# xxcclong/GNN-Computing

Hardware: AMD Instinct MI355X
Metric: aggregated edges/sec, GCN SpMM feat=128 (higher is better)
Workload: dtype f32; 1 GPU; arxiv-shaped CSR 169343x1166243 (seed 123), GCN sum, feat=128, unit weights, locality reorder applied on load (.reorder_thres_0.2), mode=balanced; num_v=169343, num_e=1166243, feat=128

## Files before the change

gnn_computing_amd/csrc/agg_gcn.hip:

```cpp
#include "combine.cuh"

namespace gnnagg {

template <int VEC, int GROUP, bool IS_MAX, bool LIST>
__device__ __forceinline__ void gcn_items_body(const GcnArgs &a)
{
    constexpr int ITEMS = block_of<GROUP>() / GROUP;
    const int b = logical_block(blockIdx.x, a.nblocks, a.ntiles, a.remap, a.xr);
    if (b < 0) return;
    const int tile = b % a.ntiles;
    const int item = (b / a.ntiles) * ITEMS + (int)threadIdx.x / GROUP;
    const int lane = threadIdx.x & (GROUP - 1);
    const int col = (tile * GROUP + lane) * VEC;
    if (item >= a.n_total) return;
    const bool col_ok = col < a.feat;
    const int F = a.feat;

    if (LIST && item >= a.n_items) {
        const float z[VEC] = {};
        if (col_ok) store_pack<VEC>(a.y + (size_t)a.empty_rows[item - a.n_items] * F + col, z);
        return;
    }
    const int beg = a.ptr[item], end = a.ptr[item + 1];
    float acc[VEC];
// ... 119 lines not shown
    const int F = a.feat;
    const int slot = ~d.z;
    if (grp == 0 && col_ok) store_pack_wt<VEC>(a.partial, a.partial_bytes, (size_t)slot * F + col, acc);
    asm volatile("s_waitcnt vmcnt(0) lgkmcnt(0)" ::: "memory");
    __shared__ int s_hub;
    __syncthreads();
    if (threadIdx.x == 0) {
        const int m = a.slot_hub[slot];
        const int nseg = a.mrow_ptr[m + 1] - a.mrow_ptr[m];
        int *cnt = a.hub_count + (size_t)m * a.hub_count_stride + tile;
        const int old = __hip_atomic_fetch_add(cnt, 1, __ATOMIC_RELAXED, __HIP_MEMORY_SCOPE_AGENT);
        if (old == nseg - 1) __hip_atomic_store(cnt, 0, __ATOMIC_RELAXED, __HIP_MEMORY_SCOPE_AGENT);
        s_hub = old == nseg - 1 ? m : -1;
    }
    __syncthreads();
    const int m = s_hub;
    if (m < 0) return false;
    const int s0 = a.mrow_ptr[m], s1 = a.mrow_ptr[m + 1];
    const int row = a.mrow_id[m];
    row_out = row;
#pragma unroll
    for (int k = 0; k < VEC; ++k) acc[k] = IS_MAX ? -INFINITY : 0.0f;
    for (int sb = s0; sb < s1; sb += kSegChunks) {
        const int nst = s1 - sb < kSegChunks ? s1 - sb : kSegChunks;
        for (int p = grp; p < nst; p += GPB)
            if (col_ok) {
                const Pack<VEC> v = load_pack_sc1<VEC>(a.partial, a.partial_bytes, (size_t)(sb + p) * F + col);
                store_pack<VEC>(&stage[(p * GROUP + lane) * VEC], v.v);
            }
        __syncthreads();
        if (grp == 0 && col_ok) {
#pragma unroll
            for (int p = 0; p < kSegChunks; ++p)
                if (p < nst) {
                    const Pack<VEC> v = load_pack<VEC>(&stage[(p * GROUP + lane) * VEC]);
#pragma unroll
                    for (int k = 0; k < VEC; ++k) {
                        if (IS_MAX) acc[k] = v.v[k] > acc[k] ? v.v[k] : acc[k];
                        else acc[k] += v.v[k];
                    }
                }
        }
        __syncthreads();
    }
    if (grp == 0 && col_ok) {
        finish_gcn_row<VEC, IS_MAX>(acc, a.mean ? a.row_ptr[row + 1] - a.row_ptr[row] : 1, row, a.y + (size_t)row * F + col, a.mean,
                                    a.accumulate, a.relu, a.row_aux, TYPED ? a.yvec : VEC);
        if constexpr (TYPED) store_y_typed<VEC>(a.y, a.y_bf16, a.yvec, 0, 0, (size_t)row * F + col, acc);
        else store_pack<VEC>(a.y + (size_t)row * F + col, acc);
    }
    return true;
}

#ifdef GNNAGG_PLAN_WAVES
#define PLAN_WAVES_ATTR __attribute__((amdgpu_waves_per_eu(GNNAGG_PLAN_WAVES, GNNAGG_PLAN_WAVES)))
#else
#define PLAN_WAVES_ATTR
#endif
template <int VEC, int GROUP, bool IS_MAX, bool PROBE = false, int UNROLL = kUnroll, typename TX = float, bool TYPED = false>
__global__ __launch_bounds__(block_of<GROUP>()) PLAN_WAVES_ATTR void k_gcn_plan(const PlanArgs a)
{
    static_assert(TYPED || std::is_same<TX, float>::value, "16-bit X needs the typed store");
    constexpr int GPB = block_of<GROUP>() / GROUP;
    const int F = a.feat;
    const int lane = threadIdx.x & (GROUP - 1);
    const int grp = (int)threadIdx.x / GROUP;
    const int nb1 = a.n1 * a.ntiles;
    if (PROBE && (int)blockIdx.x < nb1) {
        const int tile = (int)blockIdx.x % a.ntiles;
        const int4 d = a.t1[(int)blockIdx.x / a.ntiles];
        const int col = (tile * GROUP + lane) * VEC;
        const int nch = (d.y - d.x + a.chunk - 1) / a.chunk;
        unsigned sig = 0;
        for (int c = grp; c < nch; c += GPB) {
            const int cb = d.x + c * a.chunk;
            const int ce = cb + a.chunk < d.y ? cb + a.chunk : d.y;
            sig ^= probe_edges<VEC, GROUP, UNROLL>(cb, ce, lane, col < F, a.idx, a.val, a.x + col, F);
        }
        if (sig == 0x9e3779b9u) a.probe_sink[0] = sig;
        return;
    }
    if ((int)blockIdx.x < nb1) {
        __shared__ float stage[kSegChunks * GROUP * VEC];
        const int tile = (int)blockIdx.x % a.ntiles;
        const int4 d = a.t1[(int)blockIdx.x / a.ntiles];
        const int col = (tile * GROUP + lane) * VEC;
        const bool col_ok = col < F;
        const int nch = (d.y - d.x + a.chunk - 1) / a.chunk;
        for (int c = grp; c < nch; c += GPB) {
            float acc[VEC];
#pragma unroll
            for (int k = 0; k < VEC; ++k) acc[k] = IS_MAX ? -INFINITY : 0.0f;
            const int cb = d.x + c * a.chunk;
            const int ce = cb + a.chunk < d.y ? cb + a.chunk : d.y;
            chain_edges<VEC, GROUP, IS_MAX, UNROLL, TX>(acc, cb, ce, lane, col_ok, a.idx, a.val, reinterpret_cast<const TX *>(a.x) + col, F);
            store_pack<VEC>(&stage[(c * GROUP + lane) * VEC], acc);
        }
        __syncthreads();
        const bool hub_here = d.z < 0 && a.hub_count != nullptr;
        if (!hub_here && (grp != 0 || !col_ok)) return;
        float acc[VEC];
#pragma unroll
        for (int k = 0; k < VEC; ++k) acc[k] = IS_MAX ? -INFINITY : 0.0f;
        if (grp == 0 && col_ok) {
#pragma unroll
            for (int c = 0; c < kSegChunks; ++c)
                if (c < nch) {
                    const Pack<VEC> p = load_pack<VEC>(&stage[(c * GROUP + lane) * VEC]);
#pragma unroll
                    for (int k = 0; k < VEC; ++k) {
                        if (IS_MAX) acc[k] = p.v[k] > acc[k] ? p.v[k] : acc[k];
                        else acc[k] += p.v[k];
                    }
                }
        }
        if (hub_here) {
            int row;
            hub_arrive_and_fold<VEC, GROUP, IS_MAX, TYPED>(a, d, tile, col, col_ok, grp, lane, acc, stage, row);
        } else if (d.z >= 0) {
            finish_gcn_row<VEC, IS_MAX>(acc, d.y - d.x, d.z, a.y + (size_t)d.z * F + col, a.mean, a.accumulate, a.relu, a.row_aux,
                                        TYPED ? a.yvec : VEC);
            if constexpr (TYPED) store_y_typed<VEC>(a.y, a.y_bf16, a.yvec, 0, 0, (size_t)d.z * F + col, acc);
            else store_pack<VEC>(a.y + (size_t)d.z * F + col, acc);
        } else {
            store_pack<VEC>(a.partial + (size_t)(~d.z) * F + col, acc);
        }
        return;
    }
    const int b = a.tile_major ? logical_block_tile_major((int)blockIdx.x - nb1, a.item_blocks, a.ntiles, a.xr)
                               : logical_block((int)blockIdx.x - nb1, a.nblocks0, a.ntiles, a.remap, a.xr);
    if (b < 0) return;
    const int tile = b % a.ntiles;
    const int item = (b / a.ntiles) * GPB + grp;
    if (item >= a.n0) return;
    const int col = (tile * GROUP + lane) * VEC;
    const bool col_ok = col < F;
    const int4 d = a.t0[item];
    const TX *__restrict__ xcol = reinterpret_cast<const TX *>(a.x) + (size_t)tile * a.x_tile_stride + lane * VEC;
    if constexpr (PROBE) {
        const unsigned sig = probe_edges<VEC, GROUP, UNROLL>(d.x, d.y, lane, col_ok, a.idx, a.val, xcol, a.xpitch);
        if (sig == 0x9e3779b9u) a.probe_sink[0] = sig;
        return;
    }
    if (a.accumulate && !a.relu && d.x == d.y) return;
    float acc[VEC];
#pragma unroll
    for (int k = 0; k < VEC; ++k) acc[k] = IS_MAX ? -INFINITY : 0.0f;
    chain_edges<VEC, GROUP, IS_MAX, UNROLL, TX>(acc, d.x, d.y, lane, col_ok, a.idx, a.val, xcol, a.xpitch);
    if (!col_ok) return;
    if (d.z < 0) {
        const size_t poff = (size_t)(~d.z) * a.ppitch + lane * VEC;
        if (a.ptile_bytes) store_pack_wt<VEC>(a.partial + (size_t)tile * a.p_tile_stride, a.ptile_bytes, poff, acc);
        else store_pack<VEC>(a.partial + (size_t)tile * a.p_tile_stride + poff, acc);
        return;
    }
    if (d.x == d.y) {
#pragma unroll
        for (int k = 0; k < VEC; ++k) acc[k] = 0.0f;
        finish_gcn_row<VEC, false>(acc, 1, d.z, a.y + (size_t)d.z * F + col, 0, a.accumulate, a.relu, nullptr, TYPED ? a.yvec : VEC);
    } else {
        finish_gcn_row<VEC, IS_MAX>(acc, d.y - d.x, d.z, a.y + (size_t)d.z * F + col, a.mean, a.accumulate, a.relu, a.row_aux,
                                    TYPED ? a.yvec : VEC);
    }
    if constexpr (TYPED) store_y_typed<VEC>(a.y, a.y_bf16, a.yvec, a.wt, a.ybytes, (size_t)d.z * F + col, acc);
    else if (a.yvec < VEC || F - col < VEC) store_pack_any<VEC>(a.y + (size_t)d.z * F + col, acc, F - col, a.yvec);
    else if (a.wt) store_pack_wt<VEC>(a.y, a.ybytes, (size_t)d.z * F + col, acc);
    else store_pack<VEC>(a.y + (size_t)d.z * F + col, acc);
}

#ifndef NN_ROWS
#define NN_ROWS 16
#endif
static constexpr int kNnRows = NN_ROWS;

struct NnArgs {
    const float *weight;
    float *out;
    int n_out;
};

template <int KB, int ROWS>
__device__ __forceinline__ void tile_times_weight(const float *tile, int pitch, const int *tile_rows, const float *W, int K,
                                                  int Kw, int N, float *out)
{
    const int wave = (int)threadIdx.x >> 6, lane = (int)threadIdx.x & 63;
    const int ncb = (N + 15) >> 4;
    const int Kf = K & ~3;
    const int kq = lane >> 4;
    const __amdgpu_buffer_rsrc_t wrsrc = __builtin_amdgcn_make_buffer_rsrc(const_cast<float *>(W), 0, Kw * N * 4, 0x00020000);
    bool synced = false;
    constexpr int RH = ROWS / 16;
// ... 524 lines not shown
            if (is_max) hipLaunchKernelGGL((k_gcn_plan<VEC, GROUP, true, false, 4, TX, true>), dim3(grid), dim3(blk), 0, stream, a);
            else        hipLaunchKernelGGL((k_gcn_plan<VEC, GROUP, false, false, 4, TX, true>), dim3(grid), dim3(blk), 0, stream, a);
            return;
        }
    }
    if (is_max) hipLaunchKernelGGL((k_gcn_plan<VEC, GROUP, true, false, kUnroll, TX, true>), dim3(grid), dim3(blk), 0, stream, a);
    else        hipLaunchKernelGGL((k_gcn_plan<VEC, GROUP, false, false, kUnroll, TX, true>), dim3(grid), dim3(blk), 0, stream, a);
}

int launch_gcn_plan(const GcnPlanLaunch &L, void *stream_v)
{
    hipStream_t stream = (hipStream_t)stream_v;
    if (L.feat <= 0) return fail(GNNAGG_ERR_ARG, "feature length must be >= 1");
    if (L.tile.on && (L.n1 > 0 || L.accumulate)) return fail(GNNAGG_ERR_STATE, "internal: tiled launch with segments");
    const bool typed = L.x_dtype != GNNAGG_DTYPE_F32 || L.y_dtype != GNNAGG_DTYPE_F32;
    if (typed && (L.tile.on || L.probe || L.nn_weight || L.t0_partials))
        return fail(GNNAGG_ERR_STATE, "internal: typed launch on a path without 16-bit forms");
    const int xsize = L.x_dtype == GNNAGG_DTYPE_BF16 ? 2 : 4, ysize = L.y_dtype == GNNAGG_DTYPE_BF16 ? 2 : 4;
    const Geometry g = L.tile.on ? tile_geometry(L.tile, L.feat)
                       : typed   ? typed_geometry(L.feat, L.x, xsize)
                                 : pick_geometry(L.feat, L.x, L.y, L.partial, L.feat);
    const bool is_max = L.reduce == GNNAGG_REDUCE_MAX;
    PlanArgs a;
    a.t0 = reinterpret_cast<const int4 *>(L.t0); a.t1 = reinterpret_cast<const int4 *>(L.t1);
    a.idx = L.idx; a.val = L.val; a.x = static_cast<const float *>(L.x); a.y = static_cast<float *>(L.y); a.partial = L.partial;
    a.n0 = L.n0; a.n1 = L.n1; a.feat = L.feat; a.ntiles = g.ntiles; a.chunk = L.chunk;
    a.mean = L.reduce == GNNAGG_REDUCE_MEAN; a.remap = L.xcd_remap; a.accumulate = L.accumulate; a.relu = L.relu;
    a.row_aux = L.row_aux;
    a.slot_hub = L.slot_hub; a.mrow_ptr = L.hubs.mrow_ptr; a.mrow_id = L.hubs.mrow_id; a.row_ptr = L.row_ptr;
    a.hub_count = L.hub_count; a.hub_count_stride = L.hub_count_stride; a.partial_bytes = 0;
    a.xpitch = L.feat; a.ppitch = L.feat; a.x_tile_stride = a.p_tile_stride = g.group * g.vec;
    a.yvec = typed ? align_class(L.feat, L.y, ysize, g.vec) : g.vec;
    a.y_bf16 = L.y_dtype == GNNAGG_DTYPE_BF16 ? 1 : 0;
    a.tile_major = 0; a.item_blocks = 0; a.ptile_bytes = 0; a.probe_sink = nullptr;
    if (L.tile.on) {
        a.xpitch = L.tile.xpitch; a.x_tile_stride = L.tile.x_tile_stride; a.ppitch = L.tile.ppitch;
        a.p_tile_stride = L.tile.p_tile_stride; a.yvec = L.tile.yvec; a.tile_major = 1;
        const size_t tb = (size_t)L.hubs.n_slots * L.tile.ppitch * sizeof(float);
        a.ptile_bytes = tb < 0x7fffffffULL ? (unsigned)tb : 0u;
    }
    {
        const size_t pbytes = (size_t)L.hubs.n_slots * L.feat * sizeof(float);
        if (L.hubs.n_mrows == 0 || pbytes >= 0x7fffffffULL || g.ntiles > L.hub_count_stride) a.hub_count = nullptr;
        else a.partial_bytes = (unsigned)pbytes;
    }
    const bool hubs_in_kernel = a.hub_count != nullptr;
    {
        const size_t ybytes = (size_t)L.num_rows * L.feat * ysize;
        a.wt = (!L.accumulate && ybytes < 0x7fffffffULL && g.vec * ysize <= 16) ? 1 : 0;
        a.ybytes = (unsigned)ybytes;
    }
    const bool want_nn = L.nn_weight != nullptr;
    const bool fuse_nn = want_nn && !L.tile.on && !L.probe && g.ntiles == 1 && g.group >= 16 && !L.accumulate && !L.relu && !L.t0_partials;
    const bool u4 = L.unroll == 4 && g.vec == 4 && (g.group == 32 || g.group == 64) && !L.tile.on && !fuse_nn;
    const int blk = block_for(g.group);
    const int gpb = fuse_nn ? std::max(kNnRows, blk / g.group) : blk / g.group;
    const int item_blocks = ceil_div(a.n0, gpb);
    a.nblocks0 = item_blocks * g.ntiles;
    a.item_blocks = item_blocks;
    if (a.remap && a.nblocks0 < 64 && !a.tile_major) a.remap = 0;
    int grid0 = a.nblocks0;
    if (a.tile_major) {
        if (!L.t0_cost_prefix) return fail(GNNAGG_ERR_STATE, "internal: tiled launch without item costs");
        grid0 = 8 * fill_xcd_ranges_tile_major(L.t0_cost_prefix, a.n0, gpb, item_blocks, g.ntiles, a.xr);
    } else if (a.remap == 2) {
        if (!L.t0_cost_prefix) a.remap = 1;
        else grid0 = 8 * fill_xcd_ranges(L.t0_cost_prefix, a.n0, gpb, item_blocks, a.xr) * g.ntiles;
    }
    const int grid = a.n1 * g.ntiles + grid0;
    if (typed) {
        if (grid > 0) {
            const bool u4t = L.unroll == 4 && g.vec * xsize == 16 && g.group >= 32;
#define CALL_TYPED(TXT) launch_plan_typed<VEC, GROUP, TXT>(a, is_max, u4t, grid, blk, stream)
            if (L.x_dtype == GNNAGG_DTYPE_BF16) {
                DISPATCH_GEOM_16BIT(g, CALL_TYPED(__bf16))
            } else {
                DISPATCH_GEOM(g, CALL_TYPED(float))
            }
#undef CALL_TYPED
            HIP_TRY(hipGetLastError());
        }
        if (hubs_in_kernel) return GNNAGG_OK;
        GcnLaunch C;
        C.wl = L.hubs; C.row_ptr = L.row_ptr; C.y = static_cast<float *>(L.y); C.partial = L.partial; C.feat = L.feat; C.reduce = L.reduce;
        C.accumulate = L.accumulate; C.relu = L.relu; C.row_aux = L.row_aux;
        if (L.y_dtype == GNNAGG_DTYPE_F32) return launch_combine_gcn(C, pick_geometry(L.feat, L.partial, L.y, nullptr, L.feat), is_max, stream);
        const int cv = align_class(L.feat, L.y, ysize, 4);
        return launch_combine_gcn(C, Geometry{cv, 64, ceil_div(L.feat, 64 * cv)}, is_max, stream, nullptr, nullptr, 0, nullptr, true);
    }
    if (L.probe) {
        if (is_max) return fail(GNNAGG_ERR_ARG, "probe: sum/mean only");
        a.probe_sink = device_probe_sink();
        if (!a.probe_sink) return fail(GNNAGG_ERR_HIP, "probe: no sink");
        if (grid > 0) {
#define CALL_PROBE hipLaunchKernelGGL((k_gcn_plan<VEC, GROUP, false, true>), dim3(grid), dim3(blk), 0, stream, a);
            if (u4 && g.group == 32) hipLaunchKernelGGL((k_gcn_plan<4, 32, false, true, 4>), dim3(grid), dim3(blk), 0, stream, a);
            else if (u4) hipLaunchKernelGGL((k_gcn_plan<4, 64, false, true, 4>), dim3(grid), dim3(blk), 0, stream, a);
            else DISPATCH_GEOM(g, CALL_PROBE)
#undef CALL_PROBE
            HIP_TRY(hipGetLastError());
        }
        return GNNAGG_OK;
    }
    if (fuse_nn) {
        NnArgs w;
        w.weight = L.nn_weight; w.out = L.nn_out; w.n_out = L.nn_cols;
        if (grid > 0) {
#define CALL_PLAN_NN                                                                                                 \
            if (is_max) hipLaunchKernelGGL((k_gcn_plan_nn<VEC, GROUP, true>), dim3(grid), dim3(blk), 0, stream, a, w);     \
            else        hipLaunchKernelGGL((k_gcn_plan_nn<VEC, GROUP, false>), dim3(grid), dim3(blk), 0, stream, a, w);
            DISPATCH_GEOM(g, CALL_PLAN_NN)
#undef CALL_PLAN_NN
            HIP_TRY(hipGetLastError());
        }
        GcnLaunch C;
        C.wl = L.hubs; C.row_ptr = L.row_ptr; C.y = static_cast<float *>(L.y); C.partial = L.partial; C.feat = L.feat; C.reduce = L.reduce;
        if (hubs_in_kernel) return GNNAGG_OK;
        return launch_combine_gcn(C, g, is_max, stream, L.nn_weight, L.nn_out, L.nn_cols);
    }
    if (grid > 0) {
#define CALL_PLAN                                                                                            \
        if (is_max) hipLaunchKernelGGL((k_gcn_plan<VEC, GROUP, true>), dim3(grid), dim3(blk), 0, stream, a);        \
        else        hipLaunchKernelGGL((k_gcn_plan<VEC, GROUP, false>), dim3(grid), dim3(blk), 0, stream, a);
        if (u4 && g.group == 32) {
            if (is_max) hipLaunchKernelGGL((k_gcn_plan<4, 32, true, false, 4>), dim3(grid), dim3(blk), 0, stream, a);
            else        hipLaunchKernelGGL((k_gcn_plan<4, 32, false, false, 4>), dim3(grid), dim3(blk), 0, stream, a);
        } else if (u4) {
            if (is_max) hipLaunchKernelGGL((k_gcn_plan<4, 64, true, false, 4>), dim3(grid), dim3(blk), 0, stream, a);
            else        hipLaunchKernelGGL((k_gcn_plan<4, 64, false, false, 4>), dim3(grid), dim3(blk), 0, stream, a);
        } else DISPATCH_GEOM(g, CALL_PLAN)
#undef CALL_PLAN
        HIP_TRY(hipGetLastError());
    }
    GcnLaunch C;
    C.wl = L.hubs; C.row_ptr = L.row_ptr; C.y = static_cast<float *>(L.y); C.partial = L.partial; C.feat = L.feat; C.reduce = L.reduce;
    C.accumulate = L.accumulate; C.relu = L.relu; C.row_aux = L.row_aux;
    const int rc = hubs_in_kernel ? GNNAGG_OK : launch_combine_gcn(C, g, is_max, stream, nullptr, nullptr, 0, &L.tile);
    if (rc || !want_nn) return rc;
    return launch_dense_nn(static_cast<const float *>(L.y), L.nn_weight, L.nn_out, L.num_rows, L.nn_cols, L.feat, stream);
}

int launch_gcn_rows_long(const GcnRowsLongLaunch &L, void *stream_v)
{
    hipStream_t stream = (hipStream_t)stream_v;
    if (L.n1 <= 0) return GNNAGG_OK;
    auto aligned = [](const void *p, size_t al) { return ((uintptr_t)p % al) == 0; };
    int vec = 1;
    if (L.feat % 4 == 0 && aligned(L.x, 16)) vec = 4;
    else if (L.feat % 2 == 0 && aligned(L.x, 8)) vec = 2;
    RowsLongArgs a;
    a.r1 = reinterpret_cast<const int4 *>(L.r1); a.idx = L.idx; a.val = L.val; a.x = L.x; a.y = L.y;
    a.n1 = L.n1; a.feat = L.feat; a.ntiles = ceil_div(L.feat, 32); a.mean = L.reduce == GNNAGG_REDUCE_MEAN; a.relu = L.relu;
    a.att = L.att; a.heads = L.heads; a.dhead = L.heads > 0 ? L.feat / L.heads : L.feat; a.slope = L.slope;
    const bool is_max = L.reduce == GNNAGG_REDUCE_MAX;
    const bool is_gat = L.att != nullptr;
    if (is_gat && (a.dhead % 32) != 0) return fail(GNNAGG_ERR_ARG, "long-row GAT kernel needs head width % 32 == 0");
    const bool wide = !L.medium && !is_gat && L.feat > 32 && (L.tile_w == 64 || (L.tile_w == 0 && (long)a.n1 * a.ntiles > 2L * device_cu_count()));
    if (wide) a.ntiles = ceil_div(L.feat, 64);
    const int grid = a.n1 * a.ntiles;
#define LAUNCH_LONG(V, B)                                                                                            \
    {                                                                                                                \
        const size_t lds = (size_t)long_round_edges<V, B>() * (2 * 32 + 2) * sizeof(float);                          \
        if (is_gat)      LAUNCH_LONG_K((k_gcn_rows_long<V, false, true, B>), B)                                      \
        else if (is_max) LAUNCH_LONG_K((k_gcn_rows_long<V, true, false, B>), B)                                      \
        else             LAUNCH_LONG_K((k_gcn_rows_long<V, false, false, B>), B)                                     \
    }
#define LAUNCH_WIDE(V)                                                                                               \
    {                                                                                                                \
        const size_t lds = (size_t)long_round_edges<V, kLongBlock, 64>() * (2 * 64 + 2) * sizeof(float);             \
        if (is_max) LAUNCH_LONG_K((k_gcn_rows_long<V, true, false, kLongBlock, 64>), kLongBlock)                     \
        else        LAUNCH_LONG_K((k_gcn_rows_long<V, false, false, kLongBlock, 64>), kLongBlock)                    \
    }
#define LAUNCH_LONG_K(K, B)                                                                                          \
    {                                                                                                                \
        static OncePerDevice big_lds_ok;  \
        if (lds > 64 * 1024 && big_lds_ok.first()) {                                                                 \
            HIP_TRY(hipFuncSetAttribute(reinterpret_cast<const void *>(&K), hipFuncAttributeMaxDynamicSharedMemorySize, (int)lds)); \
            big_lds_ok.done();                                                                                       \
        }                                                                                                            \
        hipLaunchKernelGGL(K, dim3(grid), dim3(B), lds, stream, a);                                                  \
    }
    if (!L.medium && !is_gat && !wide && vec == 4) {
// ... 67 lines not shown
```

gnn_computing_amd/csrc/api.hip:

```cpp
#include <hip/hip_runtime.h>

#include <algorithm>
#include <cstdio>
#include <cstdlib>
#include <cstring>
#include <ctime>
#include <mutex>
#include <queue>
#include <set>
#include <vector>

#include "api_internal.h"

namespace gnnagg {

static thread_local std::string g_last_error;
static bool g_abort_on_error = true;

int fail(int code, const std::string &msg)
{
    g_last_error = msg;
    return code;
}

// ... 138 lines not shown
                                    h_val.empty() ? nullptr : s.h_val_s.data(), tgt.data(), keep_eid ? eid.data() : nullptr);
    ptr_s.resize((size_t)G + 1);
    tgt.resize((size_t)G);
    const int kept = ptr_s[G];
    if (keep_eid) {
        eid.resize((size_t)kept);
        int rc2 = s.eperm.upload(eid);
        if (rc2) return rc2;
        if (c->keep_h_eperm) s.h_eperm = eid;
    }
    s.h_idx_s.resize((size_t)kept);
    if (!s.h_val_s.empty()) s.h_val_s.resize((size_t)kept);
    s.h_ptr_s.swap(ptr_s);
    s.h_target.swap(tgt);
    return finalize_schedule(c, s);
}

static int build_plan_into(Ctx *c, BalancedPlan &p, int chunk, bool describe_in_sched1, double *padding_ratio)
{
    int rc = fetch_host_ptr(c);
    if (rc) return rc;
    p.reset();
    p.chunk = chunk;
    const int V = c->V;
    const long seg_edges = (long)chunk * kSegChunksHost;
    std::vector<int> t0, t1, mrow_id, mrow_ptr(1, 0), big;
    struct Seg { int beg, end, dest, row; };
    std::vector<Seg> segs;
    p.t0_cost_prefix.assign(1, 0);
    int nslots = 0;
    for (int r = 0; r < V; ++r) {
        const int beg = c->h_ptr[r], end = c->h_ptr[r + 1], deg = end - beg;
        if (deg <= chunk) {
            t0.insert(t0.end(), {beg, end, r, r});
            p.t0_cost_prefix.push_back(p.t0_cost_prefix.back() + deg + kItemCost);
        } else if (deg <= seg_edges) {
            segs.push_back({beg, end, r, r});
        } else {
            const int nseg = (int)((deg + seg_edges - 1) / seg_edges);
            for (int j = 0; j < nseg; ++j) {
                const long sb = beg + (long)j * seg_edges;
                segs.push_back({(int)sb, (int)std::min<long>(sb + seg_edges, end), ~(nslots + j), r});
            }
            if (nseg > kBigRowPartials) big.push_back((int)mrow_id.size());
            nslots += nseg;
            mrow_id.push_back(r);
            mrow_ptr.push_back(nslots);
        }
    }
    std::stable_sort(segs.begin(), segs.end(), [](const Seg &a, const Seg &b) { return a.end - a.beg > b.end - b.beg; });
    for (const Seg &sg : segs) t1.insert(t1.end(), {sg.beg, sg.end, sg.dest, sg.row});
    p.n0 = (int)(t0.size() / 4);
    p.n1 = (int)(t1.size() / 4);
    p.n_mrows = (int)mrow_id.size();
    p.n_slots = nslots;
    p.n_big = (int)big.size();
    if ((rc = p.t0.upload(t0))) return rc;
    p.h_t0 = t0;
    if ((rc = p.t1.upload(t1))) return rc;
    if ((rc = p.mrow_id.upload(mrow_id))) return rc;
    if ((rc = p.mrow_ptr.upload(mrow_ptr))) return rc;
    if ((rc = p.big_rows.upload(big))) return rc;
    {
        std::vector<int> slot_hub((size_t)nslots);
        for (size_t m = 0; m + 1 < mrow_ptr.size(); ++m)
            for (int sl = mrow_ptr[m]; sl < mrow_ptr[m + 1]; ++sl) slot_hub[sl] = (int)m;
        if ((rc = p.slot_hub.upload(slot_hub))) return rc;
    }
    if (padding_ratio) {
        long padded = 0, chunks = p.n0;
        for (const Seg &sg : segs) {
            const long nch = ((long)sg.end - sg.beg + chunk - 1) / chunk;
            padded += 8 * ((nch + 7) / 8);
            chunks += nch;
        }
        *padding_ratio = chunks > 0 ? (double)(padded + p.n0) / (double)chunks : 1.0;
    }
    if (describe_in_sched1) {
        Schedule &s = c->sched[1];
        s.reset();
        s.kind = GNNAGG_SCHED_NEIGHBOR_GROUPING;
        const int G = neighbor_grouping(c->h_ptr.data(), chunk, V, nullptr, nullptr);
        s.h_ptr_s.resize((size_t)G + 1);
        s.h_target.resize((size_t)G);
        neighbor_grouping(c->h_ptr.data(), chunk, V, s.h_ptr_s.data(), s.h_target.data());
        s.num_target = G;
    }
    p.valid = true;
    return GNNAGG_OK;
}

static int build_balanced_plan(Ctx *c, int chunk) { return build_plan_into(c, c->plan, chunk, true, nullptr); }
static int pick_chunk(const Ctx *c);
static int build_balanced_plan_keep(Ctx *c) { return build_plan_into(c, c->plan, pick_chunk(c), false, nullptr); }

#ifndef GNNAGG_SORT_ROW_BYTES
#define GNNAGG_SORT_ROW_BYTES 256
#endif
static bool wants_sorted_rows(const Ctx *c, long row_bytes) { return c->sort_window > 1 && row_bytes <= GNNAGG_SORT_ROW_BYTES; }

static int ensure_sorted_rows(Ctx *c, BalancedPlan &p)
{
    if (p.t0_sorted.p || p.n0 == 0) return GNNAGG_OK;
    const int n0 = p.n0;
    const std::vector<int> &t0 = p.h_t0;
    std::vector<int> order((size_t)n0);
// ... 625 lines not shown
        S.span_g = rb.span_g.p + s0; S.n_spans = s1 - s0; S.span_cost_prefix = rb.cost[(size_t)p].data();
        if ((rc = launch_gat_span(G, c->stream))) return rc;
    }
    if ((rc = launch_untile_y_gat(c->yt.p, c->den_t.p, y, rb.n1 > 0 ? rb.hub_mask.p : nullptr, c->V, feat, tr.spec.tile_w, ht, dhead, c->stream))) return rc;
    if (fork) HIP_TRY(hipStreamWaitEvent(c->stream, c->ev_join, 0));
    else if (rb.n1 > 0 && (rc = hub_rows(c->stream))) return rc;
    *used = true;
    return GNNAGG_OK;
}

int gcn_run(Ctx *c, const float *x, float *y, int feat, int mode, int reduce, int flags, const NnRequest *nn, int probe, int x_dtype,
            int y_dtype)
{
    const bool typed = x_dtype != GNNAGG_DTYPE_F32 || y_dtype != GNNAGG_DTYPE_F32;
    if (typed && (nn || probe)) return fail(GNNAGG_ERR_ARG, "16-bit features: run_with_nn and the gather probe are fp32 only");
    if ((flags & GNNAGG_FLAG_ACCUMULATE) && (mode != GNNAGG_MODE_BALANCED || (reduce != GNNAGG_REDUCE_SUM && !c->row_aux) || !c->use_plan))
        return fail(GNNAGG_ERR_ARG, "GNNAGG_FLAG_ACCUMULATE needs GNNAGG_MODE_BALANCED and GNNAGG_REDUCE_SUM (mean / max: gnnagg_set_row_aux first)");
    const bool aux_run = c->row_aux != nullptr && reduce != GNNAGG_REDUCE_SUM;
    if (aux_run && (mode != GNNAGG_MODE_BALANCED || !c->use_plan || nn || probe))
        return fail(GNNAGG_ERR_ARG, "gnnagg_set_row_aux applies to plain GNNAGG_MODE_BALANCED runs only");
    if (c->kind != Ctx::GCN) return fail(GNNAGG_ERR_ARG, "handle is not a GCN aggregator");
    if ((flags & GNNAGG_FLAG_RELU) && nn) return fail(GNNAGG_ERR_ARG, "GNNAGG_FLAG_RELU is not available in run_with_nn");
    if (flags & ~(GNNAGG_FLAG_ACCUMULATE | GNNAGG_FLAG_RELU)) return fail(GNNAGG_ERR_ARG, "unknown flag bits");
    if (!x || !y) return fail(GNNAGG_ERR_ARG, "null feature pointer");
    if (reduce < GNNAGG_REDUCE_SUM || reduce > GNNAGG_REDUCE_MAX) return fail(GNNAGG_ERR_ARG, "bad reduce");
    if (mode < GNNAGG_MODE_ROWS || mode > GNNAGG_MODE_BALANCED) return fail(GNNAGG_ERR_ARG, "bad mode");
    if (mode == GNNAGG_MODE_ROWS && c->fast_rows) mode = GNNAGG_MODE_BALANCED;
    if (mode == GNNAGG_MODE_SCHEDULED && c->fast_scheduled && c->sched[0].valid && sched_keeps_every_edge(c)) mode = GNNAGG_MODE_BALANCED;
    if (mode == GNNAGG_MODE_ROWS && c->opt_rows_blocked && c->tiled && c->use_plan && reduce != GNNAGG_REDUCE_MAX && !probe) {
        bool used = false;
        const int rcb = run_rows_blocked(c, x, y, feat, reduce, flags, nn, &used);
        if (rcb || used) return rcb;
    }
    Schedule *s = nullptr;
    int rc = get_sched(c, mode, &s);
    if (rc) return rc;
    const bool acc_on_partitioned = ((flags & GNNAGG_FLAG_ACCUMULATE) || aux_run || typed) && c->partitions > 0;
    const bool on_plan = (mode == GNNAGG_MODE_BALANCED && c->use_plan && (c->partitions == 0 || acc_on_partitioned)) ||
                         (mode == GNNAGG_MODE_SCHEDULED && c->plan_sched.valid);
    if (typed && !on_plan)
        return fail(GNNAGG_ERR_ARG, std::string("gnnagg_gcn_run_typed (x ") + (x_dtype == GNNAGG_DTYPE_BF16 ? "bf16" : "fp32") + ", y " +
                                        (y_dtype == GNNAGG_DTYPE_BF16 ? "bf16" : "fp32") +
                                        "): this order runs on the item kernels, which are fp32 only -- use GNNAGG_MODE_BALANCED, or a "
                                        "neighbor-grouping schedule / \"fast_scheduled\" = 1 for GNNAGG_MODE_SCHEDULED");
    if (acc_on_partitioned && !c->plan.valid && (rc = build_balanced_plan_keep(c))) return rc;
    if (on_plan) {
        BalancedPlan &p = mode == GNNAGG_MODE_BALANCED ? c->plan : c->plan_sched;
        GcnPlanLaunch P;
        P.t0 = p.t0.p; P.t1 = p.t1.p; P.n0 = p.n0; P.n1 = p.n1; P.chunk = p.chunk;
        P.t0_cost_prefix = p.t0_cost_prefix.data();
        if (wants_sorted_rows(c, (long)feat * (x_dtype == GNNAGG_DTYPE_BF16 ? 2 : 4))) {
            if ((rc = ensure_sorted_rows(c, p))) return rc;
            if (p.t0_sorted.p) { P.t0 = p.t0_sorted.p; P.t0_cost_prefix = p.t0s_cost_prefix.data(); }
        }
        P.hubs.mrow_id = p.mrow_id.p; P.hubs.mrow_ptr = p.mrow_ptr.p; P.hubs.n_mrows = p.n_mrows;
        P.hubs.n_slots = p.n_slots; P.hubs.big_rows = p.big_rows.p; P.hubs.n_big = p.n_big;
        P.row_ptr = c->d_ptr; P.idx = c->d_idx; P.val = c->d_val; P.x = x; P.y = y; P.feat = feat; P.reduce = reduce;
        P.x_dtype = x_dtype; P.y_dtype = y_dtype;
        P.xcd_remap = c->xcd_remap; P.accumulate = (flags & GNNAGG_FLAG_ACCUMULATE) ? 1 : 0; P.relu = (flags & GNNAGG_FLAG_RELU) ? 1 : 0;
        P.row_aux = aux_run ? c->row_aux : nullptr;
        P.num_rows = c->V;
        if (p.n_slots > 0) {
            if ((rc = c->partial.reserve((size_t)p.n_slots * feat))) return rc;
            P.partial = c->partial.p;
        }
        if (nn) {
            P.nn_weight = nn->weight; P.nn_out = nn->out; P.nn_cols = nn->cols;
        }
        if (p.n_mrows > 0 && c->inkernel_combine) {
            if ((rc = reserve_hub_counters(c, p.n_mrows, feat, &P.hub_count_stride))) return rc;
            P.slot_hub = p.slot_hub.p; P.hub_count = c->hub_count.p;
        }
        P.probe = probe;
        P.unroll = 4;
        return launch_gcn_plan(P, c->stream);
    }
    if (mode == GNNAGG_MODE_BALANCED && c->partitions > 0 && c->plan_part.valid && c->part_descriptors) {
        BalancedPlan &p = c->plan_part;
        TiledRun tr = plan_tiles(c, *s, x, y, feat, 4);
        const bool span_run = tr.spec.on && s->n_spans > 0;
        if (!span_run && s->gpu_built) {
            c->force_host_plan = 1;
            if ((rc = build_partitioned(c, c->partitions))) return rc;
            return gcn_run(c, x, y, feat, mode, reduce, flags, nn, probe, x_dtype, y_dtype);
        }
        if (span_run) {
            tr.spec.p_tile_stride = (long)s->num_target * tr.spec.tile_w;
            tr.partial_floats = (size_t)s->num_target * tr.spec.tile_w * tr.ntiles;
        }
        bool demoted = false;
        if ((rc = reserve_partitioned_scratch(c, tr.partial_floats, 0, tr.xt_floats, &demoted))) return rc;
        if (demoted) return gcn_run(c, x, y, feat, mode, reduce, flags, nn, probe, x_dtype, y_dtype);
        if ((rc = refresh_partitioned_val(c, s))) return rc;
        if (span_run) {
            SpanLaunch S;
            S.span_g = s->span_g.p; S.n_spans = s->n_spans; S.span_cost_prefix = s->span_cost_prefix.data();
            S.ptr_s = s->ptr_s.p; S.idx_f = s->idx_f.p; S.val_s = c->d_val ? s->val_s.p : nullptr; S.target = s->target.p;
            S.n_groups = s->num_target; S.crows = s->crows.p; S.n_crows = s->n_crows; S.rg_ptr = s->rg_ptr.p; S.rg_idx = s->rg_idx.p;
            S.empty_rows = s->empty_rows.p; S.n_empty = s->n_empty; S.row_ptr = c->d_ptr;
            S.x = x; S.x_rows = s->total_cols; S.y = y; S.partial = c->partial.p; S.feat = feat; S.reduce = reduce; S.relu = (flags & GNNAGG_FLAG_RELU) ? 1 : 0;
            S.tile = tr.spec; S.probe = probe;
            if (tr.retile) {
                if ((rc = launch_tile_x(x, c->xt.p, s->total_cols, feat, tr.spec.tile_w, c->stream))) return rc;
                S.x = c->xt.p;
            }
            if ((rc = launch_gcn_span(S, c->stream)) || !nn || probe) return rc;
// ... 835 lines not shown
```

gnn_computing_amd/csrc/api_internal.h:

```cpp
#pragma once
#include <hip/hip_runtime.h>

#include <mutex>
#include <set>
#include <string>
#include <vector>

#include "common.h"
#include "devbuf.h"

namespace gnnagg {

struct Schedule {
    bool valid = false;
    int kind = GNNAGG_SCHED_NOP;
    int num_target = 0;
    bool permuted = false;
    bool gpu_built = false;
    int n_edges_perm = 0;
    int total_cols = 0;
    int par_num = 0;
    std::vector<int> h_ptr_s, h_target, h_idx_s, h_slot, h_empty;
    std::vector<int> h_eperm;
    std::vector<float> h_val_s;
    DevBuf<int> ptr_s, target, slot, empty_rows, mrow_id, mrow_ptr, idx_s, big_rows;
    DevBuf<int> eperm;
    DevBuf<int> idx_f, span_g, crows, rg_ptr, rg_idx;
    int n_spans = 0, n_crows = 0;
    std::vector<long> span_cost_prefix;
    int n_big = 0;
    DevBuf<float> val_s;
    int n_empty = 0, n_mrows = 0, n_slots = 0;
    std::vector<long> cost_prefix;

    void reset()
    {
        valid = false;
        ptr_s.release(); target.release(); slot.release(); empty_rows.release();
        mrow_id.release(); mrow_ptr.release(); idx_s.release(); val_s.release(); big_rows.release(); eperm.release(); n_big = 0;
        idx_f.release(); span_g.release(); crows.release(); rg_ptr.release(); rg_idx.release(); n_spans = n_crows = 0;
        span_cost_prefix.clear();
        h_ptr_s.clear(); h_target.clear(); h_idx_s.clear(); h_val_s.clear(); h_slot.clear(); h_empty.clear(); h_eperm.clear();
        cost_prefix.clear();
        num_target = n_empty = n_mrows = n_slots = 0;
        permuted = gpu_built = false;
        n_edges_perm = 0;
    }
    WorkList worklist() const
    {
        WorkList w;
        w.ptr = ptr_s.p; w.target = target.p; w.slot = slot.p; w.empty_rows = empty_rows.p;
        w.n_items = num_target; w.n_empty = n_empty;
        w.mrow_id = mrow_id.p; w.mrow_ptr = mrow_ptr.p; w.n_mrows = n_mrows; w.n_slots = n_slots;
        w.big_rows = big_rows.p; w.n_big = n_big;
        return w;
    }
};

struct BalancedPlan {
    bool valid = false;
    int chunk = 64;
    int n0 = 0, n1 = 0, n_mrows = 0, n_slots = 0, n_big = 0;
    DevBuf<int> t0, t1, mrow_id, mrow_ptr, big_rows, slot_hub;
    std::vector<long> t0_cost_prefix;
    std::vector<int> h_t0;
    DevBuf<int> t0_sorted;
    std::vector<long> t0s_cost_prefix;
    void reset()
    {
        valid = false;
        t0.release(); t1.release(); mrow_id.release(); mrow_ptr.release(); big_rows.release(); slot_hub.release();
        t0_cost_prefix.clear(); h_t0.clear(); t0_sorted.release(); t0s_cost_prefix.clear();
        n0 = n1 = n_mrows = n_slots = n_big = 0;
    }
};
static constexpr int kSegChunksHost = 16;

struct RowsPlan {
    bool valid = false;
    bool medium_ok = true;
    int n0 = 0, n1 = 0, n2 = 0, long_deg = 256, med_deg = 256;
    DevBuf<int> r0, r1, r2, r1_rows;
    std::vector<long> r0_cost_prefix;
};

static constexpr int kItemCost = 2;

struct Ctx {
    enum Kind { GCN, GAT } kind;
    int V = 0, E = 0;
    const int *d_ptr = nullptr;
    const int *d_idx = nullptr;
    const float *d_val = nullptr;
    const int *row_aux = nullptr;
    hipStream_t stream = nullptr;
    std::vector<int> h_ptr;
    Schedule sched[2];
    BalancedPlan plan;
    BalancedPlan plan_sched;
    BalancedPlan plan_part;
    struct RowsBlocked {
        bool tried = false, ok = false;
        Schedule sched;
        DevBuf<int> span_g, idx_f;
        DevBuf<int> r1;
        DevBuf<unsigned char> hub_mask;
        int n1 = 0;
        std::vector<int> span0;
        std::vector<std::vector<long>> cost;
        void reset() { tried = ok = false; sched.reset(); span_g.release(); idx_f.release(); r1.release(); hub_mask.release(); n1 = 0; span0.clear(); cost.clear(); }
    } rb;
    bool keep_h_eperm = false;
    DevBuf<float> yt;
    DevBuf<float> den_t;
    int opt_rows_blocked = 1;
    int opt_hub_tile = 0;
    int opt_rows_medium = 0;
    int opt_rb_hub_edges = 0;
    RowsPlan rows_plan;
    RowsPlan rows_plan_nomed;
    hipStream_t aux_stream = nullptr;
    hipEvent_t ev_fork = nullptr, ev_join = nullptr;
    Schedule sched_edges;
    DevBuf<float> den;
    DevBuf<float> partial, partial_den;
    DevBuf<float> xt;
    DevBuf<float> att_t;
#ifdef GNNAGG_EXTRAS
    int tiled = 1;
    int opt_retile = 1;
    int use_spans = 1;
    int inkernel_combine = 1;
    int use_plan = 1;
    int part_descriptors = 1;
    int opt_part_min_deg = 96;
#else
    static constexpr int tiled = 1, opt_retile = 1, use_spans = 1, inkernel_combine = 1, use_plan = 1, part_descriptors = 1, opt_part_min_deg = 96;
#endif
    int opt_partitions = -1;
// ... 52 lines not shown
```

gnn_computing_amd/csrc/common.h:

```cpp
#pragma once
#include <cstddef>
#include <cstdint>
#include <string>

#include "../../include/gnnagg.h"

namespace gnnagg {

int fail(int code, const std::string &msg);

void reorder_csr(const int *ptr, const int *idx, const int *map, const int *rmap, int V, int *newptr, int *newidx);
int neighbor_grouping(const int *ptr, int ng, int V, int *ptr_out, int *target_out);
int locality_schedule(const int *ptr, const int *idx, const float *val, int par_num, int ng, int V, int total_v,
                      int *ptr_out, int *idx_out, float *val_out, int *target_out, int *eid_out = nullptr);
int load_graph(const char *datadir, const char *dset, const char *suffix, int shuffle, int *num_v, int *num_e,
               int **ptr_o, int **idx_o, int **rows_o, int **rrows_o);
void partition_rows(const int *ptr, int V, int nparts, int *bounds);
int halo_plan_slice(const int *ptr_slice, const int *idx_slice, int num_cols, const int *bounds, int nparts, int rank, int *lptr,
                    int *lidx, int **halo_ids_o, int *halo_counts, int *num_halo);
int halo_plan(const int *ptr, const int *idx, int V, const int *bounds, int nparts, int rank, int *lptr, int *lidx,
              int **halo_ids_o, int *halo_counts, int *num_halo);
int halo_stage_count(int world, int mode, int k);
void halo_stage_plan_recv(const long long *recv_rows, int world, int rank, int mode, int k, long long *stage_recv, int *new_of_old);
void halo_stage_plan_send(const long long *send_rows, int world, int rank, int mode, int k, long long *stage_send, int *order);

int cluster_reorder(const int *ptr, const int *idx, int V, double threshold, int num_perm, int cap, uint64_t seed,
                    int max_bucket, int *rows_out, int *num_clusters_out, int order_mode = 0, int cache_rows = 4096);


static constexpr int kBigRowPartials = 64;

struct WorkList {
    const int *ptr = nullptr;
    const int *target = nullptr;
    const int *slot = nullptr;
    const int *empty_rows = nullptr;
    int n_items = 0;
    int n_empty = 0;
    const int *mrow_id = nullptr;
    const int *mrow_ptr = nullptr;
    int n_mrows = 0;
    int n_slots = 0;
    const int *big_rows = nullptr;
    int n_big = 0;
};

struct TileSpec {
    int on = 0;
    int tile_w = 64;
    int xpitch = 0;
    long x_tile_stride = 0;
    int ppitch = 0;
    long p_tile_stride = 0;
    int yvec = 1;
};

struct GcnLaunch {
    WorkList wl;
    const int *row_ptr = nullptr;
    const int *idx = nullptr;
    const float *val = nullptr;
    const float *x = nullptr;
    float *y = nullptr;
    float *partial = nullptr;
    int feat = 0;
    int reduce = GNNAGG_REDUCE_SUM;
    int xcd_remap = 1;
    int accumulate = 0;
    const int *row_aux = nullptr;
    int relu = 0;
    void *timer = nullptr;
    int *timer_blocks_out = nullptr;
    int timer_capacity = 0;
    const long *xcd_item_cost_prefix = nullptr;
};

struct GcnPlanLaunch {
    const void *t0 = nullptr;
    const void *t1 = nullptr;
    int n0 = 0, n1 = 0, chunk = 64;
    const long *t0_cost_prefix = nullptr;
    WorkList hubs;
    const int *row_ptr = nullptr;
    const int *idx = nullptr;
    const float *val = nullptr;
    const void *x = nullptr;
    void *y = nullptr;
    int x_dtype = GNNAGG_DTYPE_F32, y_dtype = GNNAGG_DTYPE_F32;
    float *partial = nullptr;
    int feat = 0;
    int reduce = GNNAGG_REDUCE_SUM;
    int xcd_remap = 2;
    int accumulate = 0;
    const int *row_aux = nullptr;
    int relu = 0;
    int num_rows = 0;
    int t0_partials = 0;
    const int *slot_hub = nullptr;
    int *hub_count = nullptr;
    int hub_count_stride = 0;
    const float *nn_weight = nullptr;
    float *nn_out = nullptr;
    int nn_cols = 0;
    TileSpec tile;
    int probe = 0;
    int unroll = 0;
};

struct SpanLaunch {
    const int *span_g = nullptr;
    int n_spans = 0;
    const long *span_cost_prefix = nullptr;
    const int *ptr_s = nullptr;
    const int *idx_f = nullptr;
    const float *val_s = nullptr;
    const int *target = nullptr;
    int n_groups = 0;
    const int *crows = nullptr;
    int n_crows = 0;
    const int *rg_ptr = nullptr, *rg_idx = nullptr;
    const int *empty_rows = nullptr;
    int n_empty = 0;
    const int *row_ptr = nullptr;
    const float *x = nullptr;
    int x_rows = 0;
    float *y = nullptr;
    float *partial = nullptr;
    int feat = 0, reduce = GNNAGG_REDUCE_SUM, relu = 0;
    TileSpec tile;
    int probe = 0;
    int chain = 0;
};
int launch_gcn_span(const SpanLaunch &a, void *stream);
int launch_zero_words(void *p, size_t n_words, void *stream);
// ... 135 lines not shown
```

Baseline: 15.85 billion edges/s.

## Process runs of consecutive short rows per group with shuffled edge indices

Adds a host-built list of runs that pack consecutive CSR rows, up to 32 rows or a budget of about 16 edges, into one work item. A new device path loads the run's row ends and edge indices cooperatively, broadcasts them with shuffles, and writes each row as its boundary is reached. The aim is to amortise per-item overhead and use lanes better on low-degree graphs like arxiv. The cost is serialised row-finish branches inside the loop, and the u4 path is now gated on runs existing or n0 being zero.

```diff
diff --git a/gnn_computing_amd/csrc/agg_gcn.hip b/gnn_computing_amd/csrc/agg_gcn.hip
--- a/gnn_computing_amd/csrc/agg_gcn.hip
+++ b/gnn_computing_amd/csrc/agg_gcn.hip
@@ -195,12 +195,102 @@
     return true;
 }
 
+template <int VEC, int GROUP, bool IS_MAX, int UNROLL, typename TX, bool TYPED>
+__device__ __forceinline__ void run_rows(const PlanArgs &a, const int4 d, int lane, int col, bool col_ok, const TX *__restrict__ xcol)
+{
+    static_assert(GROUP >= kRunRows, "a run's row ends are one load of the group");
+    const int F = a.feat;
+    const int my_end = lane < d.w ? a.row_ptr[d.z + 1 + lane] : d.y;
+    int my_s = 0;
+    float my_w = 1.0f;
+    if (d.x + lane < d.y) {
+        my_s = a.idx[d.x + lane];
+        if (a.val) my_w = a.val[d.x + lane];
+    }
+    int r = 0, rbeg = d.x, rend = __shfl(my_end, 0, GROUP);
+    float acc[VEC];
+#pragma unroll
+    for (int k = 0; k < VEC; ++k) acc[k] = IS_MAX ? -INFINITY : 0.0f;
+    auto finish_rows = [&](int e) {
+        while (r < d.w && rend == e) {
+            const int row = d.z + r, deg = rend - rbeg;
+            if (col_ok && !(a.accumulate && !a.relu && deg == 0)) {
+                if (deg == 0) {
+#pragma unroll
+                    for (int k = 0; k < VEC; ++k) acc[k] = 0.0f;
+                    finish_gcn_row<VEC, false>(acc, 1, row, a.y + (size_t)row * F + col, 0, a.accumulate, a.relu, nullptr, TYPED ? a.yvec : VEC);
+                } else {
+                    finish_gcn_row<VEC, IS_MAX>(acc, deg, row, a.y + (size_t)row * F + col, a.mean, a.accumulate, a.relu, a.row_aux,
+                                                TYPED ? a.yvec : VEC);
+                }
+                if constexpr (TYPED) store_y_typed<VEC>(a.y, a.y_bf16, a.yvec, a.wt, a.ybytes, (size_t)row * F + col, acc);
+                else if (a.yvec < VEC || F - col < VEC) store_pack_any<VEC>(a.y + (size_t)row * F + col, acc, F - col, a.yvec);
+                else if (a.wt) store_pack_wt<VEC>(a.y, a.ybytes, (size_t)row * F + col, acc);
+                else store_pack<VEC>(a.y + (size_t)row * F + col, acc);
+            }
+#pragma unroll
+            for (int k = 0; k < VEC; ++k) acc[k] = IS_MAX ? -INFINITY : 0.0f;
+            ++r;
+            rbeg = rend;
+            rend = __shfl(my_end, r, GROUP);
+        }
+    };
+    finish_rows(d.x);
+    for (int cb = d.x; cb < d.y; cb += GROUP) {
+        int nx_s = 0;
+        float nx_w = 1.0f;
+        if (cb + GROUP + lane < d.y) {
+            nx_s = a.idx[cb + GROUP + lane];
+            if (a.val) nx_w = a.val[cb + GROUP + lane];
+        }
+        const int n = d.y - cb < GROUP ? d.y - cb : GROUP;
+        for (int j = 0; j < n; j += UNROLL) {
+            int s[UNROLL];
+            float w[UNROLL];
+            Pack<VEC, TX> xv[UNROLL];
+#pragma unroll
+            for (int u = 0; u < UNROLL; ++u) {
+                s[u] = __shfl(my_s, j + u, GROUP);
+                w[u] = __shfl(my_w, j + u, GROUP);
+            }
+#pragma unroll
+            for (int u = 0; u < UNROLL; ++u)
+                if (j + u < n && col_ok) xv[u] = load_pack<VEC>(xcol + (size_t)s[u] * a.xpitch);
+#pragma unroll
+            for (int u = 0; u < UNROLL; ++u)
+                if (j + u < n) {
+                    if (col_ok) {
+#pragma unroll
+                        for (int k = 0; k < VEC; ++k) {
+                            if (IS_MAX) {
+                                const float p = xv[u].at(k) * w[u];
+                                acc[k] = p > acc[k] ? p : acc[k];
+                            } else {
+                                acc[k] = __builtin_fmaf(xv[u].at(k), w[u], acc[k]);
+                            }
+                        }
+                    }
+                    if (cb + j + u + 1 == rend) finish_rows(rend);
+                }
+        }
+        my_s = nx_s;
+        my_w = nx_w;
+    }
+}
+
+template <int VEC, int GROUP, int UNROLL>
+__device__ __forceinline__ unsigned probe_run_rows(const PlanArgs &a, const int4 d, int lane, bool col_ok, const float *__restrict__ xcol)
+{
+    unsigned sig = lane < d.w ? (unsigned)a.row_ptr[d.z + 1 + lane] : 0u;
+    return sig ^ probe_edges<VEC, GROUP, UNROLL>(d.x, d.y, lane, col_ok, a.idx, a.val, xcol, a.xpitch);
+}
+
 #ifdef GNNAGG_PLAN_WAVES
 #define PLAN_WAVES_ATTR __attribute__((amdgpu_waves_per_eu(GNNAGG_PLAN_WAVES, GNNAGG_PLAN_WAVES)))
 #else
 #define PLAN_WAVES_ATTR
 #endif
-template <int VEC, int GROUP, bool IS_MAX, bool PROBE = false, int UNROLL = kUnroll, typename TX = float, bool TYPED = false>
+template <int VEC, int GROUP, bool IS_MAX, bool PROBE = false, int UNROLL = kUnroll, typename TX = float, bool TYPED = false, bool RUNS = false>
 __global__ __launch_bounds__(block_of<GROUP>()) PLAN_WAVES_ATTR void k_gcn_plan(const PlanArgs a)
 {
     static_assert(TYPED || std::is_same<TX, float>::value, "16-bit X needs the typed store");
@@ -280,6 +370,15 @@
     const bool col_ok = col < F;
     const int4 d = a.t0[item];
     const TX *__restrict__ xcol = reinterpret_cast<const TX *>(a.x) + (size_t)tile * a.x_tile_stride + lane * VEC;
+    if constexpr (RUNS) {
+        if constexpr (PROBE) {
+            const unsigned sig = probe_run_rows<VEC, GROUP, UNROLL>(a, d, lane, col_ok, xcol);
+            if (sig == 0x9e3779b9u) a.probe_sink[0] = sig;
+        } else {
+            run_rows<VEC, GROUP, IS_MAX, UNROLL, TX, TYPED>(a, d, lane, col, col_ok, xcol);
+        }
+        return;
+    }
     if constexpr (PROBE) {
         const unsigned sig = probe_edges<VEC, GROUP, UNROLL>(d.x, d.y, lane, col_ok, a.idx, a.val, xcol, a.xpitch);
         if (sig == 0x9e3779b9u) a.probe_sink[0] = sig;
@@ -910,7 +1009,13 @@
     }
     const bool want_nn = L.nn_weight != nullptr;
     const bool fuse_nn = want_nn && !L.tile.on && !L.probe && g.ntiles == 1 && g.group >= 16 && !L.accumulate && !L.relu && !L.t0_partials;
-    const bool u4 = L.unroll == 4 && g.vec == 4 && (g.group == 32 || g.group == 64) && !L.tile.on && !fuse_nn;
+    const bool runs = L.runs && L.n_runs > 0 && !L.t0_partials && !typed;
+    const bool u4 = L.unroll == 4 && g.vec == 4 && (g.group == 32 || g.group == 64) && !L.tile.on && !fuse_nn && (runs || L.n0 == 0);
+    if (u4 && runs) {
+        a.t0 = reinterpret_cast<const int4 *>(L.runs);
+        a.n0 = L.n_runs;
+    }
+    const long *item_cost_prefix = u4 && runs ? L.runs_cost_prefix : L.t0_cost_prefix;
     const int blk = block_for(g.group);
     const int gpb = fuse_nn ? std::max(kNnRows, blk / g.group) : blk / g.group;
     const int item_blocks = ceil_div(a.n0, gpb);
@@ -922,8 +1027,8 @@
         if (!L.t0_cost_prefix) return fail(GNNAGG_ERR_STATE, "internal: tiled launch without item costs");
         grid0 = 8 * fill_xcd_ranges_tile_major(L.t0_cost_prefix, a.n0, gpb, item_blocks, g.ntiles, a.xr);
     } else if (a.remap == 2) {
-        if (!L.t0_cost_prefix) a.remap = 1;
-        else grid0 = 8 * fill_xcd_ranges(L.t0_cost_prefix, a.n0, gpb, item_blocks, a.xr) * g.ntiles;
+        if (!item_cost_prefix) a.remap = 1;
+        else grid0 = 8 * fill_xcd_ranges(item_cost_prefix, a.n0, gpb, item_blocks, a.xr) * g.ntiles;
     }
     const int grid = a.n1 * g.ntiles + grid0;
     if (typed) {
@@ -952,8 +1057,8 @@
         if (!a.probe_sink) return fail(GNNAGG_ERR_HIP, "probe: no sink");
         if (grid > 0) {
 #define CALL_PROBE hipLaunchKernelGGL((k_gcn_plan<VEC, GROUP, false, true>), dim3(grid), dim3(blk), 0, stream, a);
-            if (u4 && g.group == 32) hipLaunchKernelGGL((k_gcn_plan<4, 32, false, true, 4>), dim3(grid), dim3(blk), 0, stream, a);
-            else if (u4) hipLaunchKernelGGL((k_gcn_plan<4, 64, false, true, 4>), dim3(grid), dim3(blk), 0, stream, a);
+            if (u4 && g.group == 32) hipLaunchKernelGGL((k_gcn_plan<4, 32, false, true, 4, float, false, true>), dim3(grid), dim3(blk), 0, stream, a);
+            else if (u4) hipLaunchKernelGGL((k_gcn_plan<4, 64, false, true, 4, float, false, true>), dim3(grid), dim3(blk), 0, stream, a);
             else DISPATCH_GEOM(g, CALL_PROBE)
 #undef CALL_PROBE
             HIP_TRY(hipGetLastError());
@@ -981,11 +1086,11 @@
         if (is_max) hipLaunchKernelGGL((k_gcn_plan<VEC, GROUP, true>), dim3(grid), dim3(blk), 0, stream, a);        \
         else        hipLaunchKernelGGL((k_gcn_plan<VEC, GROUP, false>), dim3(grid), dim3(blk), 0, stream, a);
         if (u4 && g.group == 32) {
-            if (is_max) hipLaunchKernelGGL((k_gcn_plan<4, 32, true, false, 4>), dim3(grid), dim3(blk), 0, stream, a);
-            else        hipLaunchKernelGGL((k_gcn_plan<4, 32, false, false, 4>), dim3(grid), dim3(blk), 0, stream, a);
+            if (is_max) hipLaunchKernelGGL((k_gcn_plan<4, 32, true, false, 4, float, false, true>), dim3(grid), dim3(blk), 0, stream, a);
+            else        hipLaunchKernelGGL((k_gcn_plan<4, 32, false, false, 4, float, false, true>), dim3(grid), dim3(blk), 0, stream, a);
         } else if (u4) {
-            if (is_max) hipLaunchKernelGGL((k_gcn_plan<4, 64, true, false, 4>), dim3(grid), dim3(blk), 0, stream, a);
-            else        hipLaunchKernelGGL((k_gcn_plan<4, 64, false, false, 4>), dim3(grid), dim3(blk), 0, stream, a);
+            if (is_max) hipLaunchKernelGGL((k_gcn_plan<4, 64, true, false, 4, float, false, true>), dim3(grid), dim3(blk), 0, stream, a);
+            else        hipLaunchKernelGGL((k_gcn_plan<4, 64, false, false, 4, float, false, true>), dim3(grid), dim3(blk), 0, stream, a);
         } else DISPATCH_GEOM(g, CALL_PLAN)
 #undef CALL_PLAN
         HIP_TRY(hipGetLastError());
diff --git a/gnn_computing_amd/csrc/api.hip b/gnn_computing_amd/csrc/api.hip
--- a/gnn_computing_amd/csrc/api.hip
+++ b/gnn_computing_amd/csrc/api.hip
@@ -214,6 +214,30 @@
     for (const Seg &sg : segs) t1.insert(t1.end(), {sg.beg, sg.end, sg.dest, sg.row});
     p.n0 = (int)(t0.size() / 4);
     p.n1 = (int)(t1.size() / 4);
+    {
+        int budget = kRunEdges;
+        if (const char *e = getenv("GNNAGG_RUN_EDGES")) budget = std::max(1, atoi(e));
+        std::vector<int> runs;
+        p.runs_cost_prefix.assign(1, 0);
+        int r0 = -1, nr = 0;
+        auto close = [&]() {
+            if (nr == 0) return;
+            const int beg = c->h_ptr[r0], end = c->h_ptr[r0 + nr];
+            runs.insert(runs.end(), {beg, end, r0, nr});
+            p.runs_cost_prefix.push_back(p.runs_cost_prefix.back() + (end - beg) + (long)kItemCost * nr);
+            nr = 0;
+        };
+        for (int i = 0; i < p.n0; ++i) {
+            const int r = t0[4 * i + 2];
+            if (nr > 0 && r != r0 + nr) close();
+            if (nr == 0) r0 = r;
+            ++nr;
+            if (nr == kRunRows || c->h_ptr[r0 + nr] - c->h_ptr[r0] >= budget) close();
+        }
+        close();
+        p.n_runs = (int)(runs.size() / 4);
+        if ((rc = p.runs.upload(runs))) return rc;
+    }
     p.n_mrows = (int)mrow_id.size();
     p.n_slots = nslots;
     p.n_big = (int)big.size();
@@ -945,6 +969,9 @@
         if (wants_sorted_rows(c, (long)feat * (x_dtype == GNNAGG_DTYPE_BF16 ? 2 : 4))) {
             if ((rc = ensure_sorted_rows(c, p))) return rc;
             if (p.t0_sorted.p) { P.t0 = p.t0_sorted.p; P.t0_cost_prefix = p.t0s_cost_prefix.data(); }
+        }
+        if (P.t0 == p.t0.p && p.n_runs > 0) {
+            P.runs = p.runs.p; P.n_runs = p.n_runs; P.runs_cost_prefix = p.runs_cost_prefix.data();
         }
         P.hubs.mrow_id = p.mrow_id.p; P.hubs.mrow_ptr = p.mrow_ptr.p; P.hubs.n_mrows = p.n_mrows;
         P.hubs.n_slots = p.n_slots; P.hubs.big_rows = p.big_rows.p; P.hubs.n_big = p.n_big;
diff --git a/gnn_computing_amd/csrc/api_internal.h b/gnn_computing_amd/csrc/api_internal.h
--- a/gnn_computing_amd/csrc/api_internal.h
+++ b/gnn_computing_amd/csrc/api_internal.h
@@ -63,6 +63,9 @@
     int n0 = 0, n1 = 0, n_mrows = 0, n_slots = 0, n_big = 0;
     DevBuf<int> t0, t1, mrow_id, mrow_ptr, big_rows, slot_hub;
     std::vector<long> t0_cost_prefix;
+    int n_runs = 0;
+    DevBuf<int> runs;
+    std::vector<long> runs_cost_prefix;
     std::vector<int> h_t0;
     DevBuf<int> t0_sorted;
     std::vector<long> t0s_cost_prefix;
@@ -71,7 +74,8 @@
         valid = false;
         t0.release(); t1.release(); mrow_id.release(); mrow_ptr.release(); big_rows.release(); slot_hub.release();
         t0_cost_prefix.clear(); h_t0.clear(); t0_sorted.release(); t0s_cost_prefix.clear();
-        n0 = n1 = n_mrows = n_slots = n_big = 0;
+        runs.release(); runs_cost_prefix.clear();
+        n0 = n1 = n_mrows = n_slots = n_big = n_runs = 0;
     }
 };
 static constexpr int kSegChunksHost = 16;
@@ -85,6 +89,7 @@
 };
 
 static constexpr int kItemCost = 2;
+static constexpr int kRunEdges = 16;
 
 struct Ctx {
     enum Kind { GCN, GAT } kind;
diff --git a/gnn_computing_amd/csrc/common.h b/gnn_computing_amd/csrc/common.h
--- a/gnn_computing_amd/csrc/common.h
+++ b/gnn_computing_amd/csrc/common.h
@@ -75,11 +75,16 @@
     const long *xcd_item_cost_prefix = nullptr;
 };
 
+static constexpr int kRunRows = 32;
+
 struct GcnPlanLaunch {
     const void *t0 = nullptr;
     const void *t1 = nullptr;
     int n0 = 0, n1 = 0, chunk = 64;
     const long *t0_cost_prefix = nullptr;
+    const void *runs = nullptr;
+    int n_runs = 0;
+    const long *runs_cost_prefix = nullptr;
     WorkList hubs;
     const int *row_ptr = nullptr;
     const int *idx = nullptr;
```

Measured after the change: 12.73 billion edges/s, median of 2. 0.803x the previous value.
